# simmsb/dsp-stuff

Measured on AMD Instinct MI355X. Metric: mono-channel-samples/sec through 5-node chain @128-frame blocks, higher is better.
Workload: dtype f32

## Files before the change

dsp-stuff_amd/csrc/chain_kernels.hip.h:

```cpp
#pragma once
#ifndef __HIPCC_RTC__
#include <hip/hip_runtime.h>
#include <stdint.h>
#endif

namespace dspfx {

constexpr int MAX_SLOTS = 8;
constexpr int WG = 256;

enum : int {
    K_GAIN = 0, K_BIQUAD = 1, K_LOW_PASS = 2, K_HIGH_PASS = 3, K_REVERB = 4, K_DISTORT = 5,
    K_OVERDRIVE = 6, K_CHEBYSHEV = 7, K_FIR = 8, K_ADD = 9, K_MIX = 10, K_SIGNAL_GEN = 11, K_ENVELOPE = 12
};
enum : int { G_SINE = 0, G_TRIANGLE = 1, G_SQUARE = 2, G_CONSTANT = 3 };
constexpr int G_SQUARE_OR_CONST = 4;
enum : int {
    D_HARD_CLIP = 0, D_SOFT_CLIP = 1, D_TANH = 2, D_RECIP_SOFT_CLIP = 3, D_FUZZ = 4, D_SIN = 5,
    D_ATAN = 6, D_SQUARE = 7, D_CHEBYSHEV4 = 8
};

struct SlotArgs {
    int kind;
    int mode;
// ... 25 lines not shown
    int n_slots;
    int side_hop;
    unsigned mix_stride;
    unsigned c_base;
    unsigned n_launch;
    unsigned wave_base;
    unsigned w_shift;
    unsigned w_mask;
    unsigned ld;
    unsigned pad_;
    size_t io_tile_stride;
    double hop_rc;
    double third_rc;
    int fast_div;
    int xcd_remap;
    int skip_store;
    int mp_stage;
    unsigned mp_rows_a;
    const float *mp_prev_a;
    float *mp_cur_b;
    const float *mp_prev_b;
    float *mp_mix;
    float mp_div;
    float mt_div;
    int mix_per_wave;
    unsigned *mt_tickets;
    float *mt_part2;
    float *mt_mix;
    SlotArgs slot[MAX_SLOTS];
};
// ... 27 lines not shown
                                                 unsigned tid, unsigned nthreads) {
    for (unsigned f = tid; f < nframes; f += nthreads) {
        const float acc = mix_rows_sum(part2, MIX_SLICES, nframes, f);
        mix[f] = div != 0.0f ? acc / div : acc;
    }
}
__device__ __forceinline__ void mixpipe_prologue(const ChainArgs &a) {
    const unsigned b = blockIdx.x;
    if ((a.mp_stage & 1) && b < MIX_SLICES) mix_slice_reduce(a.mp_prev_a, a.mp_cur_b, a.mp_rows_a, a.nframes, b, threadIdx.x, blockDim.x);
    else if ((a.mp_stage & 2) && b == MIX_SLICES) mix_final_reduce(a.mp_prev_b, a.mp_mix, a.nframes, a.mp_div, threadIdx.x, blockDim.x);
}

struct ColdArgs {
    float *mixpart;
    unsigned nframes, mix_stride, wave_base, n_launch;
    int xcd_remap;
    float mt_div;
    int mix_per_wave;
    unsigned *mt_tickets;
    float *mt_part2, *mt_mix;
};
__device__ __forceinline__ ColdArgs cold_args() {
    typedef const __attribute__((address_space(4))) ChainArgs *KernArgPtr;
    KernArgPtr ka = (KernArgPtr)__builtin_amdgcn_kernarg_segment_ptr();
    asm volatile("" : "+s"(ka));
    ColdArgs c;
    c.mixpart = ka->mixpart;
    c.nframes = ka->nframes;
    c.mix_stride = ka->mix_stride;
    c.wave_base = ka->wave_base;
    c.n_launch = ka->n_launch;
    c.xcd_remap = ka->xcd_remap;
    c.mt_div = ka->mt_div;
    c.mix_per_wave = ka->mix_per_wave;
    c.mt_tickets = ka->mt_tickets;
    c.mt_part2 = ka->mt_part2;
    c.mt_mix = ka->mt_mix;
    return c;
}
typedef __attribute__((address_space(1))) unsigned dspfx_gu32;
__device__ __forceinline__ float ld_sc1(const float *p) {
    return __uint_as_float(__hip_atomic_load((const dspfx_gu32 *)reinterpret_cast<const unsigned *>(p), __ATOMIC_RELAXED, __HIP_MEMORY_SCOPE_AGENT));
}
__device__ __forceinline__ void st_sc1(float *p, float v) {
#ifdef DSPFX_BUS_FENCE
    *p = v;
#else
// ... 102 lines not shown
constexpr int sig(int kind, int mode = 0, int hop = 0) { return kind | (mode << 8) | (hop << 16); }
constexpr int sig_kind(int s) { return s & 0xff; }
constexpr int sig_mode(int s) { return (s >> 8) & 0xff; }
constexpr int sig_hop(int s) { return (s >> 16) & 1; }
template <int KIND> constexpr bool sig_is(int s) { return s >= 0 && sig_kind(s) == KIND; }

#ifndef DSPFX_NT
#define DSPFX_NT 15
#endif
template <int CPL> struct NVecT;
template <> struct NVecT<1> { using type = float; };
template <> struct NVecT<2> { typedef float type __attribute__((ext_vector_type(2))); };
template <> struct NVecT<4> { typedef float type __attribute__((ext_vector_type(4))); };

constexpr int S_IN = 1, S_RING_LD = 2, S_RING_ST = 4, S_OUT = 8, S_STATE = 0;
constexpr bool nt_for(int stream) { return (DSPFX_NT & stream) != 0; }

#define DSPFX_GLOBAL __attribute__((address_space(1)))
template <int CPL, bool NT>
__device__ __forceinline__ void load_vec_raw(const float *p, float (&v)[CPL]) {
    using V = typename NVecT<CPL>::type;
    const DSPFX_GLOBAL V *gp = (const DSPFX_GLOBAL V *)reinterpret_cast<const V *>(p);
    V t;
    if constexpr (NT) t = __builtin_nontemporal_load(gp);
    else t = *gp;
    if constexpr (CPL == 1) { v[0] = t; }
    else {
#pragma unroll
        for (int j = 0; j < CPL; ++j) v[j] = t[j];
    }
}
// ... 273 lines not shown
    g.g0 = tab[0];
    return g;
}
__device__ __forceinline__ float *ring_row(const SlotArgs &s, const Ctx &cx, const RingGroups &g, int f) {
    unsigned r = s.pos + cx.f0 + f;
    r = r >= s.D ? r - s.D : r;
    const unsigned gi = __builtin_amdgcn_readfirstlane(r >> 7);
    float *gb = gi == g.gia ? g.ga : (gi == g.gia + 1 ? g.gb : g.g0);
    return uniform_ptr(gb + cx.ring_base0 + (size_t)(r & 127u) * cx.ld);
}
constexpr unsigned ROW_OOB = 0x80000000u;
constexpr int BUF_AUX_NT = 2;
__device__ __forceinline__ __amdgpu_buffer_rsrc_t row_rsrc(const float *base) {
    return __builtin_amdgcn_make_buffer_rsrc(const_cast<float *>(base), 0, 0x7fffffff, 0x00020000);
}
template <int CPL, int STREAM>
__device__ __forceinline__ void load_row(__amdgpu_buffer_rsrc_t r, unsigned voff, unsigned soff, float (&v)[CPL]) {
    static_assert(CPL == 1 || CPL == 2 || CPL == 4, "one, two or four channels per lane");
    constexpr int aux = nt_for(STREAM) ? BUF_AUX_NT : 0;
    if constexpr (CPL == 1) {
        v[0] = __uint_as_float(__builtin_amdgcn_raw_buffer_load_b32(r, (int)voff, (int)soff, aux));
    } else if constexpr (CPL == 2) {
        const dspfx_u32x2 t = __builtin_amdgcn_raw_buffer_load_b64(r, (int)voff, (int)soff, aux);
        v[0] = __uint_as_float(t.x);
        v[1] = __uint_as_float(t.y);
    } else {
        const dspfx_u32x4 t = __builtin_amdgcn_raw_buffer_load_b128(r, (int)voff, (int)soff, aux);
        v[0] = __uint_as_float(t.x);
        v[1] = __uint_as_float(t.y);
        v[2] = __uint_as_float(t.z);
        v[3] = __uint_as_float(t.w);
    }
}
template <int CPL, int STREAM>
__device__ __forceinline__ void store_row(__amdgpu_buffer_rsrc_t r, unsigned voff, unsigned soff, const float (&v)[CPL]) {
    constexpr int aux = nt_for(STREAM) ? BUF_AUX_NT : 0;
    if constexpr (CPL == 1) {
        __builtin_amdgcn_raw_buffer_store_b32(__float_as_uint(v[0]), r, (int)voff, (int)soff, aux);
    } else if constexpr (CPL == 2) {
        dspfx_u32x2 t;
        t.x = __float_as_uint(v[0]);
        t.y = __float_as_uint(v[1]);
        __builtin_amdgcn_raw_buffer_store_b64(t, r, (int)voff, (int)soff, aux);
    } else {
        dspfx_u32x4 t;
        t.x = __float_as_uint(v[0]);
        t.y = __float_as_uint(v[1]);
        t.z = __float_as_uint(v[2]);
        t.w = __float_as_uint(v[3]);
        __builtin_amdgcn_raw_buffer_store_b128(t, r, (int)voff, (int)soff, aux);
    }
// ... 506 lines not shown
        }
    }
    return f;
}
template <int F>
__device__ __forceinline__ bool mixbus_lane_writes(int lane) {
    int n = F, mask = 0;
#pragma unroll
    for (int o = 32; o >= 1; o >>= 1) {
        if (n > 1) n /= 2;
        else mask |= o;
    }
    return (lane & mask) == 0;
}

__device__ __forceinline__ unsigned work_block(int remap) {
    const unsigned b = blockIdx.x, nb = gridDim.x;
    if (!remap || (nb & 7u)) return b;
    return (b & 7u) * (nb >> 3) + (b >> 3);
}

#define DSPFX_FOR_SLOTS(M) M(0) M(1) M(2) M(3) M(4) M(5) M(6) M(7)

template <int... SIGS> struct SigList {
    static constexpr int v[MAX_SLOTS] = {SIGS...};
};

constexpr unsigned MIX_SEG = 128;
struct MixStage {
    float row[2][WG / 64][MIX_SEG];
};
template <int F, int CPL>
__device__ __forceinline__ void mixbus_partial(MixStage &ms, const float (&v)[F][CPL], bool live, unsigned f0, int lane, int wave) {
    static_assert(MIX_SEG % F == 0, "a chunk never straddles two segments");
// ... 39 lines not shown
        else dst[f] = t;
    }
}
template <int CPL, class ARGS>
__device__ __forceinline__ int mixbus_live_waves(const ARGS &a, size_t wg_rel, int waves) {
    const size_t left = a.n_launch > wg_rel ? a.n_launch - wg_rel : 0;
    const size_t n = (left + 64 * CPL - 1) / (64 * CPL);
    return n < (size_t)waves ? (int)n : waves;
}
template <int F, int CPL>
__device__ __forceinline__ void mixbus_after_chunk(const ChainArgs &hot, MixStage &ms, unsigned f0) {
    const unsigned end = f0 + F;
    if (end % MIX_SEG != 0 && end != hot.nframes) return;
    const ColdArgs a = cold_args();
    const unsigned len = end % MIX_SEG ? end % MIX_SEG : MIX_SEG;
    const unsigned wb = blockDim.x == WG ? work_block(a.xcd_remap) : blockIdx.x;
    const int nw = mixbus_live_waves<CPL>(a, (size_t)wb * blockDim.x * CPL, (int)(blockDim.x / 64));
    const bool per_wave = a.mix_per_wave && blockDim.x == WG;
    mixbus_flush(a, ms, end - len, len, a.wave_base + (per_wave ? wb * (WG / 64) : wb), nw, __builtin_amdgcn_readfirstlane(threadIdx.x >> 6), threadIdx.x & 63, per_wave);
}
__device__ __forceinline__ void mix_tail_rows(unsigned wb, int wave, int lane) {
    const ColdArgs a = cold_args();
    if (!a.mt_tickets) return;
    if (a.mix_per_wave && blockDim.x == WG) mix_tail(a.wave_base + wb * (WG / 64) + (unsigned)wave, lane);
    else if (wave == 0) mix_tail(a.wave_base + wb, lane);
}

template <int F, int CPL, class SL, bool MOD = false>
__device__ __forceinline__ void chain_chunk(const ChainArgs &a, float (&st)[MAX_SLOTS][4][CPL], size_t c, const WaveAddr &w,
                                            unsigned f0, int lane, MixStage &ms, int wave) {
    float v[F][CPL];
#pragma unroll
    for (int f = 0; f < F; ++f) load_row<CPL, S_IN>(row_rsrc(a.in + w.io_base0 + (size_t)f0 * a.ld), w.io_off, (unsigned)f * (a.ld * 4u), v[f]);
    const Ctx cx{c, a.N, w.io_base0, w.io_off, w.ring_base0, w.ring_off, a.ld, f0, a.hop_div, a.hop_rc, a.third_rc, a.side, a.side_hop, true};
    RingPre<F, CPL> pre[MAX_SLOTS];
#define DSPFX_PF(I) if constexpr (sig_is<K_REVERB>(SL::v[I])) ring_prefetch<F, CPL, false>(a.slot[I], cx, pre[I]);
    DSPFX_FOR_SLOTS(DSPFX_PF)
#undef DSPFX_PF
#define DSPFX_RUN(I)                                                                 \
    if constexpr (sig_is<K_REVERB>(SL::v[I])) {                                      \
        if constexpr (sig_hop(SL::v[I])) apply_hop<F, CPL, true>(v, cx.hop_div, cx.hop_rc); \
        ring_apply<F, CPL, false>(a.slot[I], v, pre[I], cx);                         \
    } else {                                                                         \
        run_slot<SL::v[I], F, CPL, false, true, MOD>(a.slot[I], v, st[I], cx);       \
    }
    DSPFX_FOR_SLOTS(DSPFX_RUN)
#undef DSPFX_RUN
#pragma unroll
    for (int f = 0; f < F; ++f)
        if (!a.skip_store) store_row<CPL, S_OUT>(row_rsrc(a.out + w.io_base0 + (size_t)f0 * a.ld), w.io_off, (unsigned)f * (a.ld * 4u), v[f]);
    if (a.mixpart) mixbus_partial<F, CPL>(ms, v, true, f0, lane, wave);
}

#ifdef DSPFX_TS_TRACE
constexpr unsigned WG_TRACE_WAVES = 32768;
static __device__ unsigned long long dspfx_wg_trace[WG_TRACE_WAVES * 3];
#define DSPFX_WG_IN const unsigned long long wg_t_in = wall_clock64();
#define DSPFX_WG_OUT(WB, WAVE)                                                                                      \
    {                                                                                                               \
        __builtin_amdgcn_s_waitcnt(0);                                                                              \
        const unsigned wi = (WB) * (WG / 64) + (WAVE);                                                              \
        if (lane == 0 && wi < WG_TRACE_WAVES) {                                                                     \
            dspfx_wg_trace[wi * 3] = wg_t_in;                                                                       \
            dspfx_wg_trace[wi * 3 + 1] = wall_clock64();                                                            \
            dspfx_wg_trace[wi * 3 + 2] = ((unsigned long long)__builtin_amdgcn_s_getreg((31 << 11) | 20) << 32) |  \
                                         (unsigned)__builtin_amdgcn_s_getreg((31 << 11) | 4);                      \
        }                                                                                                           \
    }
#else
#define DSPFX_WG_IN
#define DSPFX_WG_OUT(WB, WAVE)
#endif
template <int F, int CPL, class SL, bool MOD = false>
__global__ void __launch_bounds__(WG) chain_kernel(const ChainArgs a) {
    DSPFX_WG_IN
    __shared__ MixStage ms;
    if (a.mp_stage) mixpipe_prologue(a);
    const unsigned wb = work_block(a.xcd_remap);
    const unsigned tid = wb * WG + threadIdx.x;
    const int lane = threadIdx.x & 63, wave = __builtin_amdgcn_readfirstlane(threadIdx.x >> 6);
    const size_t rel = (size_t)tid * CPL;
    if (rel >= a.n_launch) return;
    const size_t c = a.c_base + rel;
    float st[MAX_SLOTS][4][CPL];
#define DSPFX_LD(I) load_state<SL::v[I], CPL, false>(a.slot[I], st[I], c, a.N, true);
    DSPFX_FOR_SLOTS(DSPFX_LD)
#undef DSPFX_LD
    const WaveAddr w = wave_addr(a, c);
    unsigned f0 = 0;
    for (; f0 + F <= a.nframes; f0 += F) {
        chain_chunk<F, CPL, SL, MOD>(a, st, c, w, f0, lane, ms, wave);
        if (a.mixpart) mixbus_after_chunk<F, CPL>(a, ms, f0);
    }
    if constexpr (F > 1)
        for (; f0 < a.nframes; ++f0) {
            chain_chunk<1, CPL, SL, MOD>(a, st, c, w, f0, lane, ms, wave);
            if (a.mixpart) mixbus_after_chunk<1, CPL>(a, ms, f0);
        }
#define DSPFX_ST(I)                                                                              \
    if constexpr (sig_is<K_SIGNAL_GEN>(SL::v[I])) signal_gen_close_block<CPL>(a.slot[I], st[I], a.nframes); \
    store_state<SL::v[I], CPL, false>(a.slot[I], st[I], c, a.N, true);
    DSPFX_FOR_SLOTS(DSPFX_ST)
#undef DSPFX_ST
    DSPFX_WG_OUT(wb, wave)
    if (a.mt_tickets) mix_tail_rows(work_block(a.xcd_remap), wave, lane);
}

#ifdef DSPFX_TS_TRACE
constexpr unsigned TS_TRACE_GROUPS = 4096, TS_TRACE_STAMPS = 16;
static __device__ unsigned long long dspfx_ts_trace[TS_TRACE_GROUPS * 4 * TS_TRACE_STAMPS];
#define DSPFX_TS_STAMP(k)                                                                                          \
    if (lane == 0 && group < TS_TRACE_GROUPS) dspfx_ts_trace[((size_t)group * 4 + q) * TS_TRACE_STAMPS + (k)] = wall_clock64();
#else
#define DSPFX_TS_STAMP(k)
#endif
template <class SL> constexpr int ts_first_stateful() {
    for (int i = 0; i < MAX_SLOTS; ++i)
        if (SL::v[i] != SIG_NONE && !sig_is<K_REVERB>(SL::v[i]) && kind_nstate(sig_kind(SL::v[i])) > 0) return i;
    return MAX_SLOTS;
}
// ... 89 lines not shown
            store_row<CPL, S_OUT>(r_out, io_voff, (unsigned)f * row_bytes, v[f]);
            __builtin_amdgcn_sched_barrier(0);
        }
    DSPFX_TS_STAMP(13)
    if (a.mixpart) mixbus_partial<S, CPL>(ms, v, active, f_begin, lane, 0);
    DSPFX_TS_STAMP(14)
}

template <int S, int CPL, class SL, bool GUARD = false>
__global__ void __launch_bounds__(WG) chain_ts_kernel(const ChainArgs a) {
    __shared__ float lds_st[4][CPL][64];
    __shared__ MixStage ms;
    if (a.mp_stage) mixpipe_prologue(a);
    const int lane = threadIdx.x & 63;
    const int q = __builtin_amdgcn_readfirstlane(threadIdx.x >> 6);
    const unsigned group = work_block(a.xcd_remap);
    const unsigned wave_global = a.wave_base + group;
    const size_t rel = ((size_t)group * 64 + lane) * CPL;
    bool active = true;
    if constexpr (GUARD) active = rel < a.n_launch;
    else if (rel >= a.n_launch) return;
    DSPFX_TS_STAMP(0)
    const size_t c = a.c_base + (active ? rel : 0);
    const WaveAddr w = wave_addr(a, c);
    const unsigned f_begin = (unsigned)q * S;
    const Ctx cx{c, a.N, w.io_base0, w.io_off, w.ring_base0, w.ring_off, a.ld, f_begin, a.hop_div, a.hop_rc, a.third_rc, a.side, a.side_hop, active};
    float v[S][CPL];
    {
        const unsigned io_voff = (GUARD && !active) ? ROW_OOB : w.io_off, row_bytes = a.ld * 4u;
        const __amdgpu_buffer_rsrc_t r_in = row_rsrc(a.in + w.io_base0 + (size_t)f_begin * a.ld);
#pragma unroll
// ... 41 lines not shown
            }
        row += ns;
    }
#pragma unroll
    for (int f = 0; f < F; ++f)
        if (!a.skip_store)
            store_row<CPL, S_OUT>(row_rsrc(a.out + w.io_base0 + (size_t)f0 * a.ld), (GUARD && !active) ? ROW_OOB : w.io_off, (unsigned)f * (a.ld * 4u), v[f]);
    if (a.mixpart) mixbus_partial<F, CPL>(ms, v, !GUARD || active, f0, lane, wave);
}

template <int F, int CPL, bool GUARD, bool MOD, bool LIBM>
__global__ void __launch_bounds__(WG) chain_dyn_kernel(const ChainArgs a) {
    extern __shared__ float lds[];
    __shared__ MixStage ms;
    if (a.mp_stage) mixpipe_prologue(a);
    const unsigned wb = blockDim.x == WG ? work_block(a.xcd_remap) : blockIdx.x;
    const unsigned tid = wb * blockDim.x + threadIdx.x;
    const int lane = threadIdx.x & 63, wave = __builtin_amdgcn_readfirstlane(threadIdx.x >> 6);
    const size_t rel = (size_t)tid * CPL;
    const bool active = rel < a.n_launch;
    if (!GUARD && !active) return;
    const size_t c = a.c_base + (active ? rel : 0);
    {
        int row = 0;
#pragma unroll 1
        for (int s = 0; s < a.n_slots; ++s) {
            const int ns = slot_nstate<SIG_DYN>(a.slot[s]), np = slot_npersist<SIG_DYN>(a.slot[s]);
            for (int k = 0; k < ns; ++k) {
                float t[CPL];
#pragma unroll
                for (int j = 0; j < CPL; ++j) t[j] = 0.0f;
// ... 62 lines not shown
```

dsp-stuff_amd/csrc/dspfx.hip:

```cpp
#include "engine.h"

using namespace dspfx;
using namespace dspfx_host;

namespace dspfx_host {

thread_local const dspfx_engine *tl_err_engine = nullptr;
thread_local std::string tl_err;

int fail(dspfx_engine *e, int code, const char *fmt, ...) {
    if (e) {
        char buf[512];
        va_list ap;
        va_start(ap, fmt);
        vsnprintf(buf, sizeof buf, fmt, ap);
        va_end(ap);
        tl_err = buf;
        tl_err_engine = e;
        std::lock_guard<std::mutex> lk(e->err_mu);
        e->err = buf;
    }
    return code;
}

// ... 257 lines not shown
    a.in = src;
    a.side = c.side;
    a.out = c.out;
    a.N = N;
    a.nframes = nframes;
    a.w_shift = lay.w_shift;
    a.w_mask = lay.w_mask;
    a.ld = lay.ld;
    a.io_tile_stride = lay.tile_stride;
    a.hop_div = e->hop_div;
    a.hop_rc = 1.0 / (double)e->hop_div;
    a.third_rc = 1.0 / 3.0;
    a.fast_div = st.fast_div ? 1 : 0;
    const bool xcd_env = e->env.xcd_remap >= 0;
    a.xcd_remap = xcd_env ? e->env.xcd_remap : 1;
    a.n_slots = st.count;
    a.skip_store = (st.count == 0 && src == c.out) ? 1 : 0;
    a.side_hop = 0;
    if (e->desc.link_flags & DSPFX_LINK_INTERNAL) a.side_hop = (e->desc.link_flags & DSPFX_LINK_SIDE_RAW) ? 2 : 3;
    int rows = 0;
    for (int k = 0; k < st.count; ++k) {
        const Node &nk = e->nodes[st.first + k];
        if (nk.d.kind == DSPFX_REVERB && (!nk.d_groups || nk.groups.size() < ring_groups_for(nk.D) || !nk.D))
            return fail(e, DSPFX_ERR_STATE, "REVERB node %d has no delay ring (an allocation failed earlier)", st.first + k);
        fill_slot(e, c, st.first + k, k < MAX_SLOTS ? a.slot[k] : ga.more[k - MAX_SLOTS]);
        rows += state_rows(nk);
    }
    if (st.async || st.async_mod) adopt_async_jit(e, st);
    const Variant *tail = nullptr, *v = stage_kernel(e, c, st, &tail);
    if (st.var_ts && v == st.var && nframes == 4u * (uint32_t)st.var_ts->ts) {
        v = st.var_ts;
        if (!xcd_env) a.xcd_remap = 0;
    }
    const uint32_t per_wave = 64u * v->cpl;
    const bool whole_guard = v->ts && v->cpl == 1 && N < 32768u && st.var_ts_tail && tail == e->tail && N % per_wave && !c.window_n &&
                             nframes == 4u * (uint32_t)st.var_ts_tail->ts;
    const uint32_t n_main = whole_guard ? 0u : N - N % per_wave;
    const uint32_t waves_main = n_main / per_wave;
    const unsigned grid_main = v->ts ? waves_main : (waves_main * 64 + WG - 1) / WG;
    const bool rows_per_wave = !v->ts && N <= TS_MAX_CHANNELS;
    a.mix_per_wave = rows_per_wave ? 1 : 0;
    const unsigned rows_main = (v->ts || rows_per_wave) ? waves_main : grid_main;
    a.mix_stride = rows_main + (N - n_main + 63) / 64;
    FirMixPipe mp;
    if (bus)
        if (const int rc = bus_begin(e, c, a.mix_stride, &a.mixpart, &mp)) return rc;
    const bool tail_bus = bus && c.bus == BUS_NOW && e->mt_tickets && nframes % 2u == 0 && e->env.mix_tail != 0;
    if (tail_bus) {
// ... 12 lines not shown
            a.mp_mix = mp.mix;
            a.mp_div = mp.div;
        } else {
            if (mp.stage & 2) {
                launch_mix_reduce_final(mp.prev_b, mp.mix, nframes, stream);
                if (mp.div != 0.0f) launch_mix_finish(mp.mix, nframes, mp.div, stream);
            }
            if (mp.stage & 1) launch_mix_reduce_slices(mp.prev_a, mp.cur_b, nframes, mp.rows_a, stream);
        }
    }
    const uint32_t w0 = c.window_n ? c.window_c0 : 0u, w1 = c.window_n ? std::min(n_main, c.window_c0 + c.window_n) : n_main;
    if (w1 > w0) {
        a.c_base = w0;
        a.n_launch = w1 - w0;
        a.wave_base = (v->ts || rows_per_wave) ? w0 / per_wave : w0 / (per_wave * (WG / 64));
        ProfScope ps(e, si, stream);
        if (launch_variant(v, a, v->ts ? (w1 - w0) / per_wave : ((w1 - w0) / v->cpl + WG - 1) / WG, WG, (unsigned)(rows * WG * v->cpl * sizeof(float)), stream)) {
            if (tail_bus) (void)hipMemsetAsync(e->mt_tickets, 0, (MIX_SLICES + 1) * sizeof(unsigned), stream);
            return fail(e, DSPFX_ERR_HIP, "kernel launch failed");
        }
    }
    a.mp_stage = 0;
    if ((N % per_wave || whole_guard) && (!c.window_n || c.window_c0 + c.window_n >= N)) {
        const uint32_t n_tail = N - n_main;
        a.c_base = n_main;
        a.n_launch = n_tail;
        a.wave_base = rows_main;
        if (st.var_ts_tail && tail == e->tail && nframes == 4u * (uint32_t)st.var_ts_tail->ts) {
            a.xcd_remap = 0;
            if (whole_guard) {
                ProfScope ps(e, si, stream);
                (void)launch_variant(st.var_ts_tail, a, (n_tail + 63) / 64, WG, 0, stream);
            } else {
                (void)launch_variant(st.var_ts_tail, a, (n_tail + 63) / 64, WG, 0, stream);
            }
        } else {
            (void)launch_variant(tail, a, (n_tail + 63) / 64, 64, (unsigned)(rows * WG * sizeof(float)), stream);
        }
    }
    const hipError_t lerr = hipGetLastError();
    if (lerr != hipSuccess) {
        if (tail_bus) (void)hipMemsetAsync(e->mt_tickets, 0, (MIX_SLICES + 1) * sizeof(unsigned), stream);
        return fail(e, DSPFX_ERR_HIP, "kernel launch failed: %s", hipGetErrorString(lerr));
    }
// ... 846 lines not shown
    }
    s.ctl_off = c.ctl_off + off;
    return s;
}

static int process_block(dspfx_engine *e, const BlockCall &c, bool pieces = false) {
    const uint32_t piece = pieces ? sub_block_frames(e, c.n_frames) : c.n_frames;
    for (uint32_t p0 = 0; p0 < c.n_frames; p0 += piece) {
        const uint32_t pn = std::min(piece, c.n_frames - p0);
        if (e->has_fuzz && pn % DSPFX_BUF_SIZE)
            return fail(e, DSPFX_ERR_INVALID, "Fuzz is block-global over 128 frames: n_frames %u %% 128 != 0", pn);
        uint32_t sub = sub_block_frames(e, pn);
        if (const uint32_t tsb = ts_sub_block(e, c))
            if (pn > tsb && pn % tsb == 0 && sub >= tsb && sub % tsb == 0) sub = tsb;
        for (uint32_t f0 = p0; f0 < p0 + pn; f0 += sub) {
            const BlockCall s = sub_block(e, c, f0, std::min(sub, p0 + pn - f0));
            if (const int rc = run_subblock(e, s)) return rc;
            e->frames_submitted += s.n_frames;
        }
    }
    return DSPFX_OK;
}

int dspfx_host::check_block(dspfx_engine *e, const void *in, const void *out, uint32_t n_frames) {
    if (!in || !out) return fail(e, DSPFX_ERR_INVALID, "in/out must not be null");
    if (n_frames > e->desc.max_frames)
        return fail(e, DSPFX_ERR_INVALID, "n_frames %u > max_frames %u", n_frames, e->desc.max_frames);
    return DSPFX_OK;
}

extern "C" int dspfx_process(dspfx_engine *e, const float *in, const float *side, float *out, float *mix,
                             uint32_t n_frames, void *stream) {
    if (!e) return DSPFX_ERR_INVALID;
// ... 229 lines not shown
```

dsp-stuff_amd/csrc/engine.h:

```cpp
#pragma once
#include "../../include/dspfx.h"

#include <hip/hip_runtime.h>
#include <hip/hiprtc.h>
#include <dlfcn.h>

#include <algorithm>
#include <cmath>
#include <cstdarg>
#include <cstddef>
#include <cstdio>
#include <cstdlib>
#include <cstring>
#include <deque>
#include <atomic>
#include <chrono>
#include <map>
#include <mutex>
#include <condition_variable>
#include <deque>
#include <atomic>
#include <thread>
#include <memory>
#include <string>
// ... 40 lines not shown
    int device = 0, n_slots = 0;
    int sigs[dspfx::MAX_SLOTS];
    bool want_std = false, want_mod = false, want_ts = false, want_tail = false;
    int f_std = 16, f_mod = 8, cpl_std = 1, cpl_ts = 1;
    const JitKernel *k_std = nullptr, *k_mod = nullptr, *k_ts = nullptr, *k_tail = nullptr;
    std::string headers_dir;
    std::string cache_dir;
};

struct Pref {
    int f = -1, cpl = -1, stat = -1;
};

struct EnvSwitches {
    int xcd_remap = -1;
    int mix_tail = -1;
    int fast_div = -1;
    int jit = -1, jit_async = -1;
    int ts_tail = -1;
    int host_part = -1;
    int host_pipeline = -1;
    int menu_ring_reserve = -1;
    bool has_variant = false;
    int variant_ts = -1;
    bool variant_static0 = false;
    Pref pref;
    std::string headers_dir;
    std::string cache_dir;
};
EnvSwitches read_env_switches();
// ... 23 lines not shown
    float *out = nullptr, *mix = nullptr;
    uint32_t n_frames = 0;
    uint32_t tile_frames = 0;
    hipStream_t stream = nullptr;
    const float *xin[GRAPH_IO] = {};
    float *xout[GRAPH_IO] = {};
    const dspfx_ctl *ctl = nullptr;
    int n_ctl = 0;
    size_t ctl_off = 0;
    BusForm bus = BUS_NOW;
    float div = 0.0f;
    float *partials = nullptr;
    float *pipe_mix = nullptr;
    uint32_t window_c0 = 0, window_n = 0;
    bool window_last = true;

    BlockCall(const float *in_, const float *side_, float *out_, float *mix_, uint32_t n_frames_, hipStream_t s)
        : in(in_), side(side_), out(out_), mix(mix_), n_frames(n_frames_), tile_frames(n_frames_), stream(s) {}
    bool wants_bus() const { return mix || bus != BUS_NOW; }
    const float *signal(int node, int k) const {
        const float *s = nullptr;
        for (int i = 0; i < n_ctl; ++i)
            if (ctl[i].node == node && ctl[i].param == k) s = ctl[i].signal + ctl_off;
        return s;
    }
};

}
using namespace dspfx_host;

// ... 32 lines not shown
    mutable bool jit_unavailable = false;
    uint64_t div_n = 0;
    float div_v = 0.0f;
    bool profiling = false;
    std::vector<std::vector<std::pair<hipEvent_t, hipEvent_t>>> prof;
    std::vector<hipEvent_t> ev_pool;
    mutable std::recursive_mutex api_mu;
    int api_depth = 0;
    mutable std::mutex pend_mu;
    struct Store { uint64_t seq; int node, param; float value; };
    std::deque<Store> pending;
    std::vector<int> pub_kinds;
    std::deque<dspfx_param_event> log;
    uint64_t next_seq = 1;
    uint64_t frames_submitted = 0;
    hipStream_t cur_stream = nullptr;
    bool cur_stream_set = true;
    hipEvent_t ev_order = nullptr;
    std::mutex alloc_mu, pool_mu;
    std::vector<std::vector<float *>> ring_pool;
    std::vector<void *> retired;
    struct PubReverb { float seconds = 0.0f; int mode = 0; uint32_t D = 0; size_t have = 0; bool given = false; };
    std::vector<PubReverb> pub_rev;
    uint64_t chain_gen = 0;
    mutable std::mutex err_mu;
};

namespace dspfx_host {

struct JitKernel {
// ... 45 lines not shown
    }
    ~ProfScope() {
        if (!a) return;
        (void)hipEventRecord(b, s);
        if (e->prof.size() <= stage) e->prof.resize(stage + 1);
        e->prof[stage].emplace_back(a, b);
    }
};

bool divisor_is_fast(float c, bool have_device = true, bool forced_off = false);
bool node_divisors_fast(const Node &n, bool have_device = true, bool forced_off = false);
bool stage_fast_div(const dspfx_engine *e, const Stage &st, bool have_device = true);
bool fusable(const Node &n);
int node_hop(const dspfx_engine *e, int idx);
inline const Pref &read_pref(const dspfx_engine *e) { return e->env.pref; }
void async_jit_submit(const std::shared_ptr<AsyncJit> &job);
bool async_jit_wait(const std::shared_ptr<AsyncJit> &job, int wait_ms);
int validate_node(dspfx_engine *e, const dspfx_node_desc &d);
int plan(dspfx_engine *e);
void collect_variants(std::vector<const Variant *> &out);
void adopt_async_jit(dspfx_engine *e, const Stage &st);
void request_mod_kernel(dspfx_engine *e, const Stage &st);
int ring_rows_copy(dspfx_engine *e, Node &n, uint32_t r0, uint32_t nrows, char *host, bool to_host);
inline size_t ring_groups_for(uint32_t D) { return ((size_t)D + RING_GROUP_ROWS - 1) / RING_GROUP_ROWS; }
int ring_reserve(dspfx_engine *e, int node, uint64_t gen, size_t want_groups, size_t keep_free, bool quiet, size_t max_share);
int ring_resize(dspfx_engine *e, int node, uint32_t D, hipStream_t s);
void recompute_min_delay(dspfx_engine *e);
int run_subblock(dspfx_engine *e, const BlockCall &c);
float output_divisor(dspfx_engine *e, uint64_t n_connected);
int bind_stream(dspfx_engine *e, hipStream_t s);
// ... 51 lines not shown
```

dsp-stuff_amd/csrc/graph_kernel.hip.h:

```cpp
#pragma once
#include "chain_kernels.hip.h"

namespace dspfx {

constexpr int GRAPH_SLOTS = 16;
constexpr int GRAPH_IO = 16;
struct GraphArgs {
    ChainArgs c;
    SlotArgs more[GRAPH_SLOTS - MAX_SLOTS];
    const float *xin[GRAPH_IO - 2];
    float *xout[GRAPH_IO - 1];
};
template <int I>
__host__ __device__ __forceinline__ const SlotArgs &gslot(const GraphArgs &g) {
    if constexpr (I < MAX_SLOTS) return g.c.slot[I];
    else return g.more[I - MAX_SLOTS];
}
#define DSPFX_FOR_GSLOTS(M) M(0) M(1) M(2) M(3) M(4) M(5) M(6) M(7) M(8) M(9) M(10) M(11) M(12) M(13) M(14) M(15)

template <int F, int CPL>
__device__ __forceinline__ void g_zero(float (&r)[F][CPL]) {
#pragma unroll
    for (int f = 0; f < F; ++f)
#pragma unroll
// ... 100 lines not shown
        if (m < PROG::n_out) {
            float *dst = m == 0 ? a.out : g.xout[m >= 1 ? m - 1 : 0];
#pragma unroll
            for (int f = 0; f < F; ++f)
                store_row<CPL, S_OUT>(row_rsrc(dst + w.io_base0 + (size_t)f0 * a.ld), w.io_off, (unsigned)f * (a.ld * 4u), ys[m][f]);
        }
    }
    if (a.mixpart) mixbus_partial<F, CPL>(ms, ys[0], true, f0, lane, wave);
}

template <int F, int CPL, class PROG>
__global__ void __launch_bounds__(WG) graph_kernel(const GraphArgs g) {
    const ChainArgs &a = g.c;
    __shared__ MixStage ms;
    if (a.mp_stage) mixpipe_prologue(a);
    const unsigned wb = work_block(a.xcd_remap);
    const unsigned tid = wb * WG + threadIdx.x;
    const int lane = threadIdx.x & 63, wave = __builtin_amdgcn_readfirstlane(threadIdx.x >> 6);
    const size_t rel = (size_t)tid * CPL;
    if (rel >= a.n_launch) return;
    const size_t c = a.c_base + rel;
    float st[GRAPH_SLOTS][4][CPL];
#define DSPFX_LD(I) load_state<PROG::sigs[I], CPL, false>(gslot<I>(g), st[I], c, a.N, true);
    DSPFX_FOR_GSLOTS(DSPFX_LD)
#undef DSPFX_LD
    const WaveAddr w = wave_addr(a, c);
    unsigned f0 = 0;
    for (; f0 + F <= a.nframes; f0 += F) {
        graph_chunk<F, CPL, PROG>(g, st, c, w, f0, lane, ms, wave);
        if (a.mixpart) mixbus_after_chunk<F, CPL>(a, ms, f0);
    }
// ... 15 lines not shown
```

dsp-stuff_amd/csrc/plan.hip:

```cpp
#include "engine.h"

using namespace dspfx;
using namespace dspfx_host;

namespace dspfx_host {


bool divisor_is_fast(float c, bool have_device, bool forced_off) {
    static std::mutex mu;
    static std::map<uint32_t, bool> cache;
    if (forced_off) return false;
    if (!(c == c) || c == 0.0f || std::isinf(c)) return false;
    const float ac = fabsf(c), half = ac * 0.5f;
    int ex = 0;
    const bool even_integer = ac >= 2.0f && half == floorf(half);
    const bool pow2 = frexpf(ac, &ex) == 0.5f;
    if (!even_integer || pow2) return true;
    uint32_t bits;
    memcpy(&bits, &c, 4);
    std::lock_guard<std::mutex> lk(mu);
    auto it = cache.find(bits);
    if (it != cache.end()) return it->second;
    if (!have_device) return false;
    bool done = false, ok = false;
// ... 39 lines not shown
    const Variant *v = variants_dyn(&n);
    for (int i = 0; i < n; ++i) out.push_back(v + i);
    v = variants_static3(&n);
    for (int i = 0; i < n; ++i) out.push_back(v + i);
    v = variants_static5(&n);
    for (int i = 0; i < n; ++i) out.push_back(v + i);
}

static int env_int(const char *name) {
    const char *v = getenv(name);
    return v ? atoi(v) : -1;
}
EnvSwitches read_env_switches() {
    EnvSwitches s;
    s.xcd_remap = env_int("DSPFX_XCD_REMAP");
    s.mix_tail = env_int("DSPFX_MIX_TAIL");
    s.fast_div = env_int("DSPFX_FAST_DIV");
    s.jit = env_int("DSPFX_JIT");
    s.jit_async = env_int("DSPFX_JIT_ASYNC");
    s.ts_tail = env_int("DSPFX_TS_TAIL");
    s.menu_ring_reserve = env_int("DSPFX_MENU_RING_RESERVE");
    s.host_part = env_int("DSPFX_HOST_PART");
    s.host_pipeline = env_int("DSPFX_HOST_PIPELINE");
    if (const char *v = getenv("DSPFX_VARIANT")) {
        s.has_variant = true;
        const char *q;
        if ((q = strstr(v, "f="))) s.pref.f = atoi(q + 2);
        if ((q = strstr(v, "cpl="))) s.pref.cpl = atoi(q + 4);
        if ((q = strstr(v, "static="))) s.pref.stat = atoi(q + 7);
        if ((q = strstr(v, "ts="))) s.variant_ts = atoi(q + 3);
// ... 285 lines not shown
```

dsp-stuff_amd/csrc/state_util.hip:

```cpp
#include "engine.h"

using namespace dspfx;
using namespace dspfx_host;



extern "C" int dspfx_link_average(dspfx_engine *e, const float *const *srcs, int n_srcs, float *dst, uint32_t n_frames,
                                  void *stream) {
    if (!e) return DSPFX_ERR_INVALID;
    ApiScope api(e);
    if (api.rc) return api.rc;
    if (!dst || n_srcs < 0 || (n_srcs > 0 && !srcs)) return fail(e, DSPFX_ERR_INVALID, "bad link list");
    if (n_srcs > DSPFX_MAX_LINKS) return fail(e, DSPFX_ERR_UNSUPPORTED, "more than %d links into one port", DSPFX_MAX_LINKS);
    if (n_frames == 0) return DSPFX_OK;
    if (n_frames > e->desc.max_frames) return fail(e, DSPFX_ERR_INVALID, "n_frames %u > max_frames %u", n_frames, e->desc.max_frames);
    for (int k = 0; k < n_srcs; ++k)
        if (!srcs[k]) return fail(e, DSPFX_ERR_INVALID, "link %d is null", k);
    HIPCHK(e, hipSetDevice(e->device));
    LinkAvgArgs a;
    memset(&a, 0, sizeof a);
    for (int k = 0; k < n_srcs; ++k) a.src[k] = srcs[k];
    a.n_srcs = n_srcs;
    a.dst = dst;
    a.count = (size_t)n_frames * e->desc.channels;
// ... 268 lines not shown
            size_t reserved = 0;
            {
                std::lock_guard<std::mutex> lk(const_cast<dspfx_engine *>(e)->pool_mu);
                if (i < e->ring_pool.size()) reserved = e->ring_pool[i].size();
            }
            snprintf(buf, sizeof buf, "node %zu delay ring: %u samples in %zu of %zu groups x %zu MiB (+%zu reserved), %d re-placed by the placement probe\n", i,
                     e->nodes[i].D, ring_groups_for(e->nodes[i].D), e->nodes[i].groups.size(), (e->nodes[i].group_floats * sizeof(float)) >> 20, reserved,
                     e->nodes[i].ring_replaced);
            s += buf;
            if (getenv("DSPFX_DESCRIBE_GROUPS"))
                for (size_t g = 0; g < e->nodes[i].groups.size(); ++g) {
                    snprintf(buf, sizeof buf, "  group %zu @%p\n", g, (void *)e->nodes[i].groups[g]);
                    s += buf;
                }
        }
    {
        const std::string &cdir = e->env.cache_dir;
        snprintf(buf, sizeof buf, "run-time kernels of this process: %llu compiled, %llu loaded from the disk cache, %llu written to it (%s)\n",
                 (unsigned long long)g_jit_compiled.load(), (unsigned long long)g_jit_from_disk.load(), (unsigned long long)g_jit_disk_written.load(),
                 cdir.empty() ? "no disk cache" : cdir.c_str());
        s += buf;
        const std::string rej = jit_cache_rejected();
        if (!rej.empty()) {
            snprintf(buf, sizeof buf, "note: the disk cache %s is NOT used: the directory must belong to this user and be writable by nobody else "
                                      "(chmod go-w, or point DSPFX_CACHE_DIR elsewhere); kernels are recompiled by every process\n", rej.c_str());
            s += buf;
        }
    }
    if (e->jit_unavailable)
        s += "note: a run-time specialised kernel was wanted but could not be compiled (hiprtc unavailable, or DSPFX_KERNEL_HEADERS "
// ... 5 lines not shown
```

Baseline: 373.4 billion.

## Alternate tile walk direction across launches and keep edge output rows cached

Consecutive sub-block launches now alternate between walking workgroups front-to-back and back-to-front, so the rows written last by one launch are read first by the next and may still sit in the last-level cache. Workgroups within a configurable zone (default 96 MiB) at each end of the launch store their output with temporal (cached) stores instead of non-temporal ones, so that data is retained for the following launch. The feature is on by default for standard kernels with two or more channels per lane. It adds per-launch parity state and a branch in the store path, and could hurt if the cache zone evicts other useful data or the reversal conflicts with the XCD remapping.

Result: faster. 385.6 billion (median of 6 runs) (+3.3%).

```diff
diff --git a/dsp-stuff_amd/csrc/chain_kernels.hip.h b/dsp-stuff_amd/csrc/chain_kernels.hip.h
--- a/dsp-stuff_amd/csrc/chain_kernels.hip.h
+++ b/dsp-stuff_amd/csrc/chain_kernels.hip.h
@@ -63,6 +63,8 @@
     double third_rc;
     int fast_div;
     int xcd_remap;
+    int walk_rev;
+    unsigned walk_zone;
     int skip_store;
     int mp_stage;
     unsigned mp_rows_a;
@@ -120,7 +122,7 @@
 struct ColdArgs {
     float *mixpart;
     unsigned nframes, mix_stride, wave_base, n_launch;
-    int xcd_remap;
+    int xcd_remap, walk_rev;
     float mt_div;
     int mix_per_wave;
     unsigned *mt_tickets;
@@ -137,6 +139,7 @@
     c.wave_base = ka->wave_base;
     c.n_launch = ka->n_launch;
     c.xcd_remap = ka->xcd_remap;
+    c.walk_rev = ka->walk_rev;
     c.mt_div = ka->mt_div;
     c.mix_per_wave = ka->mix_per_wave;
     c.mt_tickets = ka->mt_tickets;
@@ -269,7 +272,7 @@
 template <> struct NVecT<4> { typedef float type __attribute__((ext_vector_type(4))); };
 
 constexpr int S_IN = 1, S_RING_LD = 2, S_RING_ST = 4, S_OUT = 8, S_STATE = 0;
-constexpr bool nt_for(int stream) { return (DSPFX_NT & stream) != 0; }
+constexpr bool nt_for(int stream, int mask = DSPFX_NT) { return (mask & stream) != 0; }
 
 #define DSPFX_GLOBAL __attribute__((address_space(1)))
 template <int CPL, bool NT>
@@ -573,10 +576,10 @@
 __device__ __forceinline__ __amdgpu_buffer_rsrc_t row_rsrc(const float *base) {
     return __builtin_amdgcn_make_buffer_rsrc(const_cast<float *>(base), 0, 0x7fffffff, 0x00020000);
 }
-template <int CPL, int STREAM>
+template <int CPL, int STREAM, int NTM = DSPFX_NT>
 __device__ __forceinline__ void load_row(__amdgpu_buffer_rsrc_t r, unsigned voff, unsigned soff, float (&v)[CPL]) {
     static_assert(CPL == 1 || CPL == 2 || CPL == 4, "one, two or four channels per lane");
-    constexpr int aux = nt_for(STREAM) ? BUF_AUX_NT : 0;
+    constexpr int aux = nt_for(STREAM, NTM) ? BUF_AUX_NT : 0;
     if constexpr (CPL == 1) {
         v[0] = __uint_as_float(__builtin_amdgcn_raw_buffer_load_b32(r, (int)voff, (int)soff, aux));
     } else if constexpr (CPL == 2) {
@@ -591,9 +594,9 @@
         v[3] = __uint_as_float(t.w);
     }
 }
-template <int CPL, int STREAM>
+template <int CPL, int STREAM, int NTM = DSPFX_NT>
 __device__ __forceinline__ void store_row(__amdgpu_buffer_rsrc_t r, unsigned voff, unsigned soff, const float (&v)[CPL]) {
-    constexpr int aux = nt_for(STREAM) ? BUF_AUX_NT : 0;
+    constexpr int aux = nt_for(STREAM, NTM) ? BUF_AUX_NT : 0;
     if constexpr (CPL == 1) {
         __builtin_amdgcn_raw_buffer_store_b32(__float_as_uint(v[0]), r, (int)voff, (int)soff, aux);
     } else if constexpr (CPL == 2) {
@@ -1130,10 +1133,15 @@
     return (lane & mask) == 0;
 }
 
-__device__ __forceinline__ unsigned work_block(int remap) {
+__device__ __forceinline__ unsigned work_block(int remap, int rev) {
     const unsigned b = blockIdx.x, nb = gridDim.x;
-    if (!remap || (nb & 7u)) return b;
-    return (b & 7u) * (nb >> 3) + (b >> 3);
+    if (!remap || (nb & 7u)) return rev ? nb - 1u - b : b;
+    const unsigned per = nb >> 3, i = b >> 3;
+    return (b & 7u) * per + (rev ? per - 1u - i : i);
+}
+
+__device__ __forceinline__ bool walk_cached_out(unsigned zone) {
+    return blockIdx.x < zone || blockIdx.x + zone >= gridDim.x;
 }
 
 #define DSPFX_FOR_SLOTS(M) M(0) M(1) M(2) M(3) M(4) M(5) M(6) M(7)
@@ -1203,7 +1211,7 @@
     if (end % MIX_SEG != 0 && end != hot.nframes) return;
     const ColdArgs a = cold_args();
     const unsigned len = end % MIX_SEG ? end % MIX_SEG : MIX_SEG;
-    const unsigned wb = blockDim.x == WG ? work_block(a.xcd_remap) : blockIdx.x;
+    const unsigned wb = blockDim.x == WG ? work_block(a.xcd_remap, a.walk_rev) : blockIdx.x;
     const int nw = mixbus_live_waves<CPL>(a, (size_t)wb * blockDim.x * CPL, (int)(blockDim.x / 64));
     const bool per_wave = a.mix_per_wave && blockDim.x == WG;
     mixbus_flush(a, ms, end - len, len, a.wave_base + (per_wave ? wb * (WG / 64) : wb), nw, __builtin_amdgcn_readfirstlane(threadIdx.x >> 6), threadIdx.x & 63, per_wave);
@@ -1217,7 +1225,7 @@
 
 template <int F, int CPL, class SL, bool MOD = false>
 __device__ __forceinline__ void chain_chunk(const ChainArgs &a, float (&st)[MAX_SLOTS][4][CPL], size_t c, const WaveAddr &w,
-                                            unsigned f0, int lane, MixStage &ms, int wave) {
+                                            unsigned f0, int lane, MixStage &ms, int wave, bool out_cached) {
     float v[F][CPL];
 #pragma unroll
     for (int f = 0; f < F; ++f) load_row<CPL, S_IN>(row_rsrc(a.in + w.io_base0 + (size_t)f0 * a.ld), w.io_off, (unsigned)f * (a.ld * 4u), v[f]);
@@ -1235,9 +1243,16 @@
     }
     DSPFX_FOR_SLOTS(DSPFX_RUN)
 #undef DSPFX_RUN
-#pragma unroll
-    for (int f = 0; f < F; ++f)
-        if (!a.skip_store) store_row<CPL, S_OUT>(row_rsrc(a.out + w.io_base0 + (size_t)f0 * a.ld), w.io_off, (unsigned)f * (a.ld * 4u), v[f]);
+    if (!a.skip_store) {
+        const __amdgpu_buffer_rsrc_t r_out = row_rsrc(a.out + w.io_base0 + (size_t)f0 * a.ld);
+        if (out_cached) {
+#pragma unroll
+            for (int f = 0; f < F; ++f) store_row<CPL, S_OUT, DSPFX_NT & ~S_OUT>(r_out, w.io_off, (unsigned)f * (a.ld * 4u), v[f]);
+        } else {
+#pragma unroll
+            for (int f = 0; f < F; ++f) store_row<CPL, S_OUT>(r_out, w.io_off, (unsigned)f * (a.ld * 4u), v[f]);
+        }
+    }
     if (a.mixpart) mixbus_partial<F, CPL>(ms, v, true, f0, lane, wave);
 }
 
@@ -1265,7 +1280,7 @@
     DSPFX_WG_IN
     __shared__ MixStage ms;
     if (a.mp_stage) mixpipe_prologue(a);
-    const unsigned wb = work_block(a.xcd_remap);
+    const unsigned wb = work_block(a.xcd_remap, a.walk_rev);
     const unsigned tid = wb * WG + threadIdx.x;
     const int lane = threadIdx.x & 63, wave = __builtin_amdgcn_readfirstlane(threadIdx.x >> 6);
     const size_t rel = (size_t)tid * CPL;
@@ -1276,14 +1291,15 @@
     DSPFX_FOR_SLOTS(DSPFX_LD)
 #undef DSPFX_LD
     const WaveAddr w = wave_addr(a, c);
+    const bool out_cached = walk_cached_out(a.walk_zone);
     unsigned f0 = 0;
     for (; f0 + F <= a.nframes; f0 += F) {
-        chain_chunk<F, CPL, SL, MOD>(a, st, c, w, f0, lane, ms, wave);
+        chain_chunk<F, CPL, SL, MOD>(a, st, c, w, f0, lane, ms, wave, out_cached);
         if (a.mixpart) mixbus_after_chunk<F, CPL>(a, ms, f0);
     }
     if constexpr (F > 1)
         for (; f0 < a.nframes; ++f0) {
-            chain_chunk<1, CPL, SL, MOD>(a, st, c, w, f0, lane, ms, wave);
+            chain_chunk<1, CPL, SL, MOD>(a, st, c, w, f0, lane, ms, wave, out_cached);
             if (a.mixpart) mixbus_after_chunk<1, CPL>(a, ms, f0);
         }
 #define DSPFX_ST(I)                                                                              \
@@ -1292,7 +1308,7 @@
     DSPFX_FOR_SLOTS(DSPFX_ST)
 #undef DSPFX_ST
     DSPFX_WG_OUT(wb, wave)
-    if (a.mt_tickets) mix_tail_rows(work_block(a.xcd_remap), wave, lane);
+    if (a.mt_tickets) mix_tail_rows(work_block(a.xcd_remap, a.walk_rev), wave, lane);
 }
 
 #ifdef DSPFX_TS_TRACE
@@ -1412,7 +1428,7 @@
     if (a.mp_stage) mixpipe_prologue(a);
     const int lane = threadIdx.x & 63;
     const int q = __builtin_amdgcn_readfirstlane(threadIdx.x >> 6);
-    const unsigned group = work_block(a.xcd_remap);
+    const unsigned group = work_block(a.xcd_remap, a.walk_rev);
     const unsigned wave_global = a.wave_base + group;
     const size_t rel = ((size_t)group * 64 + lane) * CPL;
     bool active = true;
@@ -1484,7 +1500,7 @@
     extern __shared__ float lds[];
     __shared__ MixStage ms;
     if (a.mp_stage) mixpipe_prologue(a);
-    const unsigned wb = blockDim.x == WG ? work_block(a.xcd_remap) : blockIdx.x;
+    const unsigned wb = blockDim.x == WG ? work_block(a.xcd_remap, a.walk_rev) : blockIdx.x;
     const unsigned tid = wb * blockDim.x + threadIdx.x;
     const int lane = threadIdx.x & 63, wave = __builtin_amdgcn_readfirstlane(threadIdx.x >> 6);
     const size_t rel = (size_t)tid * CPL;
diff --git a/dsp-stuff_amd/csrc/dspfx.hip b/dsp-stuff_amd/csrc/dspfx.hip
--- a/dsp-stuff_amd/csrc/dspfx.hip
+++ b/dsp-stuff_amd/csrc/dspfx.hip
@@ -295,6 +295,7 @@
     a.fast_div = st.fast_div ? 1 : 0;
     const bool xcd_env = e->env.xcd_remap >= 0;
     a.xcd_remap = xcd_env ? e->env.xcd_remap : 1;
+    a.walk_rev = c.walk_rev ? 1 : 0;
     a.n_slots = st.count;
     a.skip_store = (st.count == 0 && src == c.out) ? 1 : 0;
     a.side_hop = 0;
@@ -313,6 +314,7 @@
         v = st.var_ts;
         if (!xcd_env) a.xcd_remap = 0;
     }
+    if (v->ts) a.walk_rev = 0;
     const uint32_t per_wave = 64u * v->cpl;
     const bool whole_guard = v->ts && v->cpl == 1 && N < 32768u && st.var_ts_tail && tail == e->tail && N % per_wave && !c.window_n &&
                              nframes == 4u * (uint32_t)st.var_ts_tail->ts;
@@ -355,6 +357,10 @@
         a.c_base = w0;
         a.n_launch = w1 - w0;
         a.wave_base = (v->ts || rows_per_wave) ? w0 / per_wave : w0 / (per_wave * (WG / 64));
+        if (c.walk_alt && !v->ts && v->cpl >= 2) {
+            const uint64_t wg_bytes = (uint64_t)WG * v->cpl * nframes * sizeof(float);
+            a.walk_zone = (unsigned)std::min<uint64_t>(((uint64_t)walk_zone_mib(e) << 20) / wg_bytes, 0x7fffffffu);
+        }
         ProfScope ps(e, si, stream);
         if (launch_variant(v, a, v->ts ? (w1 - w0) / per_wave : ((w1 - w0) / v->cpl + WG - 1) / WG, WG, (unsigned)(rows * WG * v->cpl * sizeof(float)), stream)) {
             if (tail_bus) (void)hipMemsetAsync(e->mt_tickets, 0, (MIX_SLICES + 1) * sizeof(unsigned), stream);
@@ -362,6 +368,7 @@
         }
     }
     a.mp_stage = 0;
+    a.walk_zone = 0;
     if ((N % per_wave || whole_guard) && (!c.window_n || c.window_c0 + c.window_n >= N)) {
         const uint32_t n_tail = N - n_main;
         a.c_base = n_main;
@@ -369,6 +376,7 @@
         a.wave_base = rows_main;
         if (st.var_ts_tail && tail == e->tail && nframes == 4u * (uint32_t)st.var_ts_tail->ts) {
             a.xcd_remap = 0;
+            a.walk_rev = 0;
             if (whole_guard) {
                 ProfScope ps(e, si, stream);
                 (void)launch_variant(st.var_ts_tail, a, (n_tail + 63) / 64, WG, 0, stream);
@@ -1245,9 +1253,13 @@
         if (const uint32_t tsb = ts_sub_block(e, c))
             if (pn > tsb && pn % tsb == 0 && sub >= tsb && sub % tsb == 0) sub = tsb;
         for (uint32_t f0 = p0; f0 < p0 + pn; f0 += sub) {
-            const BlockCall s = sub_block(e, c, f0, std::min(sub, p0 + pn - f0));
+            BlockCall s = sub_block(e, c, f0, std::min(sub, p0 + pn - f0));
+            const bool alternate = walk_alternates(e) && !s.window_n;
+            s.walk_alt = alternate;
+            s.walk_rev = alternate && (e->walk_parity & 1u);
             if (const int rc = run_subblock(e, s)) return rc;
             e->frames_submitted += s.n_frames;
+            if (alternate) e->walk_parity ^= 1u;
         }
     }
     return DSPFX_OK;
diff --git a/dsp-stuff_amd/csrc/engine.h b/dsp-stuff_amd/csrc/engine.h
--- a/dsp-stuff_amd/csrc/engine.h
+++ b/dsp-stuff_amd/csrc/engine.h
@@ -78,6 +78,8 @@
 
 struct EnvSwitches {
     int xcd_remap = -1;
+    int walk = -1;
+    int walk_zone_mib = -1;
     int mix_tail = -1;
     int fast_div = -1;
     int jit = -1, jit_async = -1;
@@ -131,6 +133,8 @@
     float *pipe_mix = nullptr;
     uint32_t window_c0 = 0, window_n = 0;
     bool window_last = true;
+    bool walk_rev = false;
+    bool walk_alt = false;
 
     BlockCall(const float *in_, const float *side_, float *out_, float *mix_, uint32_t n_frames_, hipStream_t s)
         : in(in_), side(side_), out(out_), mix(mix_), n_frames(n_frames_), tile_frames(n_frames_), stream(s) {}
@@ -193,6 +197,7 @@
     std::deque<dspfx_param_event> log;
     uint64_t next_seq = 1;
     uint64_t frames_submitted = 0;
+    uint32_t walk_parity = 0;
     hipStream_t cur_stream = nullptr;
     bool cur_stream_set = true;
     hipEvent_t ev_order = nullptr;
@@ -268,6 +273,10 @@
 bool fusable(const Node &n);
 int node_hop(const dspfx_engine *e, int idx);
 inline const Pref &read_pref(const dspfx_engine *e) { return e->env.pref; }
+constexpr bool WALK_ALTERNATES_DEFAULT = true;
+inline bool walk_alternates(const dspfx_engine *e) { return e->env.walk >= 0 ? e->env.walk != 0 : WALK_ALTERNATES_DEFAULT; }
+constexpr uint32_t WALK_ZONE_MIB = 96;
+inline uint32_t walk_zone_mib(const dspfx_engine *e) { return e->env.walk_zone_mib >= 0 ? (uint32_t)e->env.walk_zone_mib : WALK_ZONE_MIB; }
 void async_jit_submit(const std::shared_ptr<AsyncJit> &job);
 bool async_jit_wait(const std::shared_ptr<AsyncJit> &job, int wait_ms);
 int validate_node(dspfx_engine *e, const dspfx_node_desc &d);
diff --git a/dsp-stuff_amd/csrc/graph_kernel.hip.h b/dsp-stuff_amd/csrc/graph_kernel.hip.h
--- a/dsp-stuff_amd/csrc/graph_kernel.hip.h
+++ b/dsp-stuff_amd/csrc/graph_kernel.hip.h
@@ -138,7 +138,7 @@
     const ChainArgs &a = g.c;
     __shared__ MixStage ms;
     if (a.mp_stage) mixpipe_prologue(a);
-    const unsigned wb = work_block(a.xcd_remap);
+    const unsigned wb = work_block(a.xcd_remap, a.walk_rev);
     const unsigned tid = wb * WG + threadIdx.x;
     const int lane = threadIdx.x & 63, wave = __builtin_amdgcn_readfirstlane(threadIdx.x >> 6);
     const size_t rel = (size_t)tid * CPL;
diff --git a/dsp-stuff_amd/csrc/plan.hip b/dsp-stuff_amd/csrc/plan.hip
--- a/dsp-stuff_amd/csrc/plan.hip
+++ b/dsp-stuff_amd/csrc/plan.hip
@@ -77,6 +77,8 @@
 EnvSwitches read_env_switches() {
     EnvSwitches s;
     s.xcd_remap = env_int("DSPFX_XCD_REMAP");
+    s.walk = env_int("DSPFX_WALK");
+    s.walk_zone_mib = env_int("DSPFX_WALK_ZONE_MIB");
     s.mix_tail = env_int("DSPFX_MIX_TAIL");
     s.fast_div = env_int("DSPFX_FAST_DIV");
     s.jit = env_int("DSPFX_JIT");
diff --git a/dsp-stuff_amd/csrc/state_util.hip b/dsp-stuff_amd/csrc/state_util.hip
--- a/dsp-stuff_amd/csrc/state_util.hip
+++ b/dsp-stuff_amd/csrc/state_util.hip
@@ -306,6 +306,13 @@
                     s += buf;
                 }
         }
+    if (walk_alternates(e)) {
+        snprintf(buf, sizeof buf, "tile walk: consecutive launches over all channels alternate front-to-back / back-to-front; "
+                                  "standard kernels at two or more channels per lane keep %u MiB of output rows at each end of a launch in the last-level cache\n", walk_zone_mib(e));
+        s += buf;
+    } else {
+        s += "tile walk: every launch front to back\n";
+    }
     {
         const std::string &cdir = e->env.cache_dir;
         snprintf(buf, sizeof buf, "run-time kernels of this process: %llu compiled, %llu loaded from the disk cache, %llu written to it (%s)\n",
```
